# qinzheng93/GeoTransformer

Hardware: NVIDIA H100
Metric: point-cloud pairs/sec (3DMatch-shape synth) (higher is better)
Workload: dtype f32

## Files before the change

### geotransformer_b200/_lib.py

```python
import ctypes
import os
import threading

import torch

_HERE = os.path.dirname(os.path.abspath(__file__))
LIB_PATH = os.path.join(_HERE, 'libgeob200.so')
_lib = None

c_void_p, c_int64, c_int32, c_float, c_double, c_size_t, c_int = (
    ctypes.c_void_p, ctypes.c_int64, ctypes.c_int32, ctypes.c_float, ctypes.c_double, ctypes.c_size_t, ctypes.c_int)

SIGNATURES = {}


def _sig(name, restype, *argtypes):
    SIGNATURES[name] = (restype, list(argtypes))


P, I64, I32, F, D, SZ = c_void_p, c_int64, c_int32, c_float, c_double, c_size_t
_sig('geob200_last_error', ctypes.c_char_p)
_sig('geob200_launch_count', ctypes.c_uint64)
_sig('geob200_grid_subsample_workspace_bytes', SZ, I64, I64)
_sig('geob200_grid_subsample', c_int, P, I64, P, I64, F, P, P, P, SZ, P)
# ... 5 lines not shown
_sig('geob200_kpconv', c_int, P, P, P, P, I64, I64, I64, P, I64, P, P, I64, I64, F, P, P, SZ, P)
_sig('geob200_kpconv_tc_workspace_bytes', SZ, I64, I64, I64)
_sig('geob200_kpconv_tc', c_int, P, P, P, P, I64, I64, I64, P, I64, P, P, I64, I64, F, P, P, SZ, P)
_sig('geob200_set_linear_mode', None, c_int)
_sig('geob200_linear', c_int, P, I64, P, P, P, I64, I64, I64, I64, c_int, P)
_sig('geob200_split_tf32', c_int, P, I64, I64, I64, P, P)
_sig('geob200_linear_batched', c_int, P, I64, I64, P, I64, I64, P, I64, P, I64, I64, I64, I64, I64, I64, c_int, P)
_sig('geob200_group_norm_workspace_bytes', SZ, I64)
_sig('geob200_group_norm', c_int, P, I64, I64, I64, P, P, F, P, c_int, F, P, P, SZ, P)
_sig('geob200_fused_group_norm_workspace_bytes', SZ, I64, I64, I64)
_sig('geob200_linear_group_norm', c_int, P, I64, P, P, I64, I64, I64, I64, P, P, F, P, c_int, F, P, P, P, SZ, P)
_sig('geob200_kpconv_group_norm', c_int, P, P, P, P, I64, I64, I64, P, I64, P, P, I64, I64, F, I64, P, P, F, c_int, F, P, P, P, SZ,
     P, SZ, P)
_sig('geob200_group_norm_batched', c_int, P, I64, I64, I64, P, P, F, P, c_int, F, P, P, SZ, P, I64, P)
_sig('geob200_linear_group_norm_batched', c_int, P, I64, P, P, I64, I64, I64, I64, P, P, F, P, c_int, F, P, P, P, SZ, P, I64, P)
_sig('geob200_maxpool', c_int, P, P, I64, I64, I64, I64, P, P)
_sig('geob200_upsample_concat', c_int, P, P, I64, I64, P, I64, I64, I64, P, P)
_sig('geob200_kpconv_backward_workspace_bytes', SZ, I64, I64, I64, I64, I64)
_sig('geob200_kpconv_backward', c_int, P, P, P, P, I64, I64, I64, P, I64, P, I64, I64, F, P, P, P, P, P, SZ, P)
_sig('geob200_linear_backward_workspace_bytes', SZ, I64, I64, I64, c_int)
_sig('geob200_linear_backward', c_int, P, I64, P, P, I64, I64, I64, P, P, P, P, P, SZ, P)
_sig('geob200_group_norm_backward_batched_workspace_bytes', SZ, I64, I64, I64, I64)
_sig('geob200_group_norm_backward_batched', c_int, P, P, I64, I64, I64, P, F, c_int, F, P, P, P, P, P, P, SZ, P, I64, P)
_sig('geob200_maxpool_backward_batched_workspace_bytes', SZ, I64, I64, I64, I64)
_sig('geob200_maxpool_backward_batched', c_int, P, P, I64, I64, I64, I64, P, I64, P, P, P, P, SZ, P)
_sig('geob200_upsample_concat_backward_workspace_bytes', SZ, I64, I64)
_sig('geob200_upsample_concat_backward', c_int, P, I64, I64, I64, I64, I64, P, P, P, P, SZ, P)
_sig('geob200_point_to_node_partition_batched', c_int, P, P, I64, P, P, I64, P, P, P, P, P, P)
_sig('geob200_gather_rows', c_int, P, I64, I64, P, I64, P, P)
_sig('geob200_knn_partition', c_int, P, I64, P, I64, I64, P, P, P)
# ... 168 lines not shown
```

### geotransformer_b200/csrc/common.cuh

```cuda
#pragma once
#include <cuda_runtime.h>
#include <stdint.h>
#include <stdio.h>

namespace geob200 {

void set_error(const char* fmt, ...);
void count_launches(int n);
int ensure_max_smem(const void* kernel);

#define GEOB_CHECK_CUDA(expr)                                                                   \
    do {                                                                                        \
        cudaError_t _e = (expr);                                                                \
        if (_e != cudaSuccess) {                                                                \
            geob200::set_error("%s:%d CUDA error %s: %s", __FILE__, __LINE__, #expr,            \
                               cudaGetErrorString(_e));                                         \
            return -1;                                                                          \
        }                                                                                       \
    } while (0)

#define GEOB_CHECK_LAUNCH()                                                                     \
    do {                                                                                        \
        cudaError_t _e = cudaGetLastError();                                                    \
        if (_e != cudaSuccess) {                                                                \
// ... 63 lines not shown
                           int64_t n_query, int64_t n_support, int64_t n_neighbors, const float* kernel_points, int64_t n_kernel,
                           const float* weights_t, const float* bias, int64_t c_in, int64_t c_out, float sigma, int64_t groups,
                           const float* gamma, const float* beta, float eps, int leaky, float slope, float* pre_norm, float* y,
                           void* gn_workspace, size_t gn_workspace_bytes, void* workspace, size_t workspace_bytes, void* stream,
                           const GnSeg* seg, const float* w_img = nullptr);
int linear_img(const float* x, int64_t ldx, const float* weight, const float* w_img, const float* bias, float* y, int64_t ldy,
               int64_t m, int64_t n, int64_t k, int relu, void* stream);
int kpconv_tc_impl(const float* s_feats, const float* q_points, const float* s_points, const int64_t* neighbors, int64_t n_query,
                   int64_t n_support, int64_t n_neighbors, const float* kernel_points, int64_t n_kernel, const float* weights_t,
                   const float* w_img, const float* bias, int64_t c_in, int64_t c_out, float sigma, float* out, void* workspace,
                   size_t workspace_bytes, void* stream);

int maxpool_seg(const float* x, const int64_t* neighbors, int64_t n_query, int64_t n_support, int64_t n_neighbors, int64_t channels,
                float* y, const GnSeg* seg, const int* cloud_max, void* stream);

struct Segs {
    int n;
    int max;
    int start[GEOB_MAX_CLOUDS];
    int count[GEOB_MAX_CLOUDS];
};
int segs_from_counts(Segs* s, int64_t n, const int64_t* counts);
Segs segs_one(int64_t count);
Segs segs_range(const Segs& s, int first, int n);
int segs_products(Segs* s, const Segs& ref, const Segs& src);

struct Arena {
    char* base;
    size_t off;
    size_t cap;
// ... 46 lines not shown
```

### geotransformer_b200/csrc/kpconv.cu

```cuda
#include "common.cuh"
#include "geob200.h"
#include "kpconv.cuh"

namespace geob200 {

constexpr int TQ = 32;
constexpr int CC = 32;

__global__ void __launch_bounds__(256) kpconv_c1_kernel(const float* __restrict__ feats, const float* __restrict__ q_pts,
                                                        const float* __restrict__ s_pts, const long long* __restrict__ nbr,
                                                        int H, const float* __restrict__ kp, const float* __restrict__ W,
                                                        const float* __restrict__ bias, float sigma, int Ns, int M, int Cout,
                                                        float* __restrict__ out) {
    __shared__ float kp_s[KP * 3];
    __shared__ float wk_s[16][KP_PAD];
    __shared__ float np_s[16];
    if (threadIdx.x < KP * 3) kp_s[threadIdx.x] = kp[threadIdx.x];
    __syncthreads();
    const int lane = threadIdx.x & 31, warp = threadIdx.x >> 5;
    const int sub = lane >> 4, sl = lane & 15;
    const int slot = warp * 2 + sub;
    const int m = blockIdx.x * 16 + slot;
    const bool live = m < M;
    float acc[KP];
#pragma unroll
    for (int k = 0; k < KP; ++k) acc[k] = 0.f;
    int npos = 0;
    if (live) {
        const float qx = q_pts[3ll * m], qy = q_pts[3ll * m + 1], qz = q_pts[3ll * m + 2];
        for (int h = sl; h < H; h += 16) {
            const long long idx = nbr[(long long)m * H + h];
            if (idx < Ns) {
                float w[KP];
                influence15(kp_s, s_pts[3 * idx] - qx, s_pts[3 * idx + 1] - qy, s_pts[3 * idx + 2] - qz, 0.f, sigma, w);
                const float f = feats[idx];
                npos += (f > 0.f);
#pragma unroll
                for (int k = 0; k < KP; ++k) acc[k] = fmaf(w[k], f, acc[k]);
            }
        }
    }
#pragma unroll
    for (int k = 0; k < KP; ++k) {
#pragma unroll
        for (int o = 8; o > 0; o >>= 1) acc[k] += __shfl_xor_sync(0xffffffffu, acc[k], o);
    }
#pragma unroll
    for (int o = 8; o > 0; o >>= 1) npos += __shfl_xor_sync(0xffffffffu, npos, o);
    if (sl == 0) {
#pragma unroll
        for (int k = 0; k < KP; ++k) wk_s[slot][k] = acc[k];
        np_s[slot] = (float)max(npos, 1);
    }
    __syncwarp();
// ... 536 lines not shown
        sa = (red[0] + red[2]) + (red[4] + red[6]);
        sb = (red[1] + red[3]) + (red[5] + red[7]);
        const double count = (double)cpg * (double)rows;
        const double mean = sa / count;
        double var = sb / count - mean * mean;
        if (var < 0.0) var = 0.0;
        mean_rstd[((long long)p * G + g) * 2] = (float)mean;
        mean_rstd[((long long)p * G + g) * 2 + 1] = (float)(1.0 / sqrt(var + eps));
    }
}

constexpr int GN_RPB = 32;
__global__ void __launch_bounds__(256) gn_seg_apply_kernel(const float* __restrict__ x, const float* __restrict__ mean_rstd,
                                                           const float* __restrict__ gamma, const float* __restrict__ beta,
                                                           const float* __restrict__ residual, float* __restrict__ y, int n_rows,
                                                           int C, int cpg, int G, int leaky, float slope, GnSeg seg) {
    extern __shared__ float gn_tab[];
    __shared__ int starts[GEOB_MAX_CLOUDS + 1];
    for (int i = threadIdx.x; i <= seg.n_clouds; i += blockDim.x) starts[i] = seg.start[i];
    __syncthreads();
    const int r0 = blockIdx.x * GN_RPB, r1 = min(n_rows, r0 + GN_RPB);
    int c0 = 0, hi = seg.n_clouds;
    while (hi - c0 > 1) {
        const int mid = (c0 + hi) >> 1;
        if (starts[mid] <= r0) c0 = mid; else hi = mid;
    }
    for (int i = threadIdx.x; i < 2 * C; i += blockDim.x) {
        const int t = i / C, c = i % C;
        const int cl = min(c0 + t, seg.n_clouds - 1);
        const float* mr = mean_rstd + (long long)(cl % seg.n_pairs) * 2 * G + 2 * (c / cpg);
        gn_tab[(2 * t) * C + c] = mr[0];
        gn_tab[(2 * t + 1) * C + c] = mr[1];
    }
    __syncthreads();
    const int b0 = starts[c0 + 1];
    const int b1 = (c0 + 2 <= seg.n_clouds) ? starts[c0 + 2] : n_rows;
    const int C4 = C >> 2;
    const long long base4 = (long long)r0 * C4;
    const int total4 = (r1 - r0) * C4;
    for (int i = threadIdx.x; i < total4; i += blockDim.x) {
        const int row = r0 + i / C4, c = (i % C4) * 4;
        const float4 v = reinterpret_cast<const float4*>(x)[base4 + i];
        float4 rv = make_float4(0.f, 0.f, 0.f, 0.f);
        if (residual != nullptr) rv = reinterpret_cast<const float4*>(residual)[base4 + i];
        float in[4] = {v.x, v.y, v.z, v.w}, o[4];
        const float rs[4] = {rv.x, rv.y, rv.z, rv.w};
        if (row < b1) {
            const float* ta = gn_tab + (row < b0 ? 0 : 2 * C) + c;
            const float4 gm = __ldg(reinterpret_cast<const float4*>(gamma + c)), bt = __ldg(reinterpret_cast<const float4*>(beta + c));
            const float ga[4] = {gm.x, gm.y, gm.z, gm.w}, ba[4] = {bt.x, bt.y, bt.z, bt.w};
#pragma unroll
            for (int u = 0; u < 4; ++u) o[u] = (in[u] - ta[u]) * ta[C + u] * ga[u] + ba[u] + rs[u];
        } else {
            int lo = c0, hh = seg.n_clouds;
            while (hh - lo > 1) {
                const int mid = (lo + hh) >> 1;
                if (starts[mid] <= row) lo = mid; else hh = mid;
            }
            const float* mr = mean_rstd + (long long)(lo % seg.n_pairs) * 2 * G;
#pragma unroll
            for (int u = 0; u < 4; ++u) {
                const int g = (c + u) / cpg;
                o[u] = (in[u] - mr[2 * g]) * mr[2 * g + 1] * gamma[c + u] + beta[c + u] + rs[u];
            }
        }
        if (leaky) {
#pragma unroll
            for (int u = 0; u < 4; ++u) o[u] = o[u] > 0.f ? o[u] : o[u] * slope;
        }
        reinterpret_cast<float4*>(y)[base4 + i] = make_float4(o[0], o[1], o[2], o[3]);
    }
}

__global__ void __launch_bounds__(256) gn_apply_kernel(const float* __restrict__ x, const float* __restrict__ mean_rstd,
                                                       const float* __restrict__ gamma, const float* __restrict__ beta,
                                                       const float* __restrict__ residual, float* __restrict__ y,
                                                       long long total4, int C, int cpg, int leaky, float slope) {
    const long long i = (long long)blockIdx.x * blockDim.x + threadIdx.x;
    if (i >= total4) return;
    const float4 v = reinterpret_cast<const float4*>(x)[i];
    const int c = (int)((i * 4) % C);
    float in[4] = {v.x, v.y, v.z, v.w}, o[4];
    float4 rv = make_float4(0.f, 0.f, 0.f, 0.f);
    if (residual != nullptr) rv = reinterpret_cast<const float4*>(residual)[i];
    const float rs[4] = {rv.x, rv.y, rv.z, rv.w};
#pragma unroll
    for (int u = 0; u < 4; ++u) {
        const int g = (c + u) / cpg;
        float t = (in[u] - mean_rstd[2 * g]) * mean_rstd[2 * g + 1] * gamma[c + u] + beta[c + u];
        t += rs[u];
        if (leaky) t = t > 0.f ? t : t * slope;
        o[u] = t;
    }
    reinterpret_cast<float4*>(y)[i] = make_float4(o[0], o[1], o[2], o[3]);
}

__device__ __forceinline__ void maxpool_row(const float* __restrict__ x, const long long* __restrict__ nb, int W, int Ns, int C,
                                            float* __restrict__ yrow, int lane) {
    constexpr int NI = 5;
    if ((C & 3) == 0 && W <= 32 * NI) {
        int idx_l[NI];
#pragma unroll
        for (int i = 0; i < NI; ++i) idx_l[i] = (lane + 32 * i < W) ? (int)min(nb[lane + 32 * i], (long long)Ns) : Ns;
        const int C4 = C >> 2;
        for (int c0 = 0; c0 < C4; c0 += 32) {
            const int c4 = c0 + lane;
            const bool active = c4 < C4;
// ... 275 lines not shown
}

namespace geob200 {
size_t fused_group_norm_workspace_bytes_batched(int64_t n_rows, int64_t channels, int64_t groups, int64_t n_pairs) {
    return geob200_fused_group_norm_workspace_bytes(n_rows, channels, groups) + (size_t)(2 * groups * 4) * (size_t)(n_pairs > 1 ? n_pairs : 1) + 512;
}
struct GnWs { unsigned* ticket; float* mean_rstd; double* partial; };
static GnWs gn_carve(void* workspace, size_t bytes, int64_t groups, int64_t n_pairs = 1) {
    Arena ar(workspace, bytes);
    GnWs w;
    w.ticket = ar.take<unsigned>(64);
    w.mean_rstd = ar.take<float>(2 * groups * n_pairs);
    w.partial = ar.take<double>(1);
    return w;
}
static void launch_gn_seg_apply(const float* x, const GnWs& w, const float* gamma, const float* beta, const float* residual, float* y,
                                int64_t n_rows, int64_t channels, int64_t groups, float eps, int leaky, float slope, const GnSeg& seg,
                                cudaStream_t st) {
    const int cpg = (int)(channels / groups);
    const int slot_width = cpg < 32 ? cpg : 32;
    gn_seg_finalize_kernel<<<dim3((unsigned)groups, (unsigned)seg.n_pairs), 128, 0, st>>>(
        w.partial, x, (int)channels, (int)(channels / slot_width), cpg / slot_width, (int)groups, (double)eps, seg, w.mean_rstd);
    gn_seg_apply_kernel<<<(unsigned)((n_rows + GN_RPB - 1) / GN_RPB), 256, sizeof(float) * 4 * channels, st>>>(
        x, w.mean_rstd, gamma, beta, residual, y, (int)n_rows, (int)channels, cpg, (int)groups, leaky, slope, seg);
    count_launches(2);
}
static void launch_gn_tile_stats(const float* x, const GnWs& w, int64_t n_rows, int64_t channels, int64_t groups, cudaStream_t st) {
    const int cpg = (int)(channels / groups);
    const int slot_width = cpg < 32 ? cpg : 32;
    gn_tile_stats_kernel<<<(unsigned)((n_rows + 127) / 128), 256, sizeof(double) * 2 * (channels / slot_width), st>>>(
        x, (int)n_rows, (int)channels, slot_width, w.partial);
    count_launches(1);
}
static void launch_gn_apply(const float* x, const GnWs& w, const float* gamma, const float* beta, const float* residual, float* y,
                            int64_t n_rows, int64_t channels, int64_t groups, float eps, int leaky, float slope, cudaStream_t st) {
    const int cpg = (int)(channels / groups);
    const int slot_width = cpg < 32 ? cpg : 32;
    gn_finalize_kernel<<<1, 1024, 0, st>>>(w.partial, (int)((n_rows + 127) / 128), (int)(channels / slot_width), cpg / slot_width,
                                           (int)groups, (double)cpg * (double)n_rows, (double)eps, w.mean_rstd);
    const long long total4 = n_rows * channels / 4;
    gn_apply_kernel<<<(unsigned)((total4 + 255) / 256), 256, 0, st>>>(x, w.mean_rstd, gamma, beta, residual, y, total4, (int)channels,
                                                                     (int)(channels / groups), leaky, slope);
}
}

extern "C" {

int geob200_group_norm(const float* x, int64_t n_rows, int64_t channels, int64_t groups, const float* gamma,
                       const float* beta, float eps, const float* residual, int leaky, float slope, float* y,
                       void* workspace, size_t workspace_bytes, void* stream) {
    return geob200::group_norm_impl(x, n_rows, channels, groups, gamma, beta, eps, residual, leaky, slope, y, workspace, workspace_bytes,
                                    stream, nullptr);
}
}

namespace geob200 {
int group_norm_impl(const float* x, int64_t n_rows, int64_t channels, int64_t groups, const float* gamma, const float* beta, float eps,
// ... 216 lines not shown

int geob200_kpconv_group_norm_batched(const float* s_feats, const float* q_points, const float* s_points, const int64_t* neighbors,
                                      int64_t n_query, int64_t n_support, int64_t n_neighbors, const float* kernel_points, int64_t n_kernel,
                                      const float* weights_t, const float* bias, int64_t c_in, int64_t c_out, float sigma, int64_t groups,
                                      const float* gamma, const float* beta, float eps, int leaky, float slope, float* pre_norm, float* y,
                                      void* gn_workspace, size_t gn_workspace_bytes, void* workspace, size_t workspace_bytes, void* stream,
                                      int64_t n_pairs, const int64_t* cloud_rows_h) {
    geob200::GnSeg seg;
    if (geob200::make_seg(&seg, n_pairs, cloud_rows_h, n_query, "kpconv_group_norm")) return -2;
    GEOB_REQUIRE(pre_norm != nullptr && y != nullptr, "kpconv_group_norm: null output");
    return geob200::kpconv_group_norm_impl(s_feats, q_points, s_points, neighbors, n_query, n_support, n_neighbors, kernel_points, n_kernel,
                                           weights_t, bias, c_in, c_out, sigma, groups, gamma, beta, eps, leaky, slope, pre_norm, y,
                                           gn_workspace, gn_workspace_bytes, workspace, workspace_bytes, stream, &seg);
}

int geob200_maxpool_batched(const float* x, const int64_t* neighbors, int64_t n_query, int64_t n_support, int64_t n_neighbors,
                            int64_t channels, const int32_t* cloud_max, int64_t n_pairs, const int64_t* cloud_rows_h, float* y,
                            void* stream) {
    geob200::GnSeg seg;
    if (geob200::make_seg(&seg, n_pairs, cloud_rows_h, n_query, "maxpool")) return -2;
    GEOB_REQUIRE(n_query > 0 && n_support > 0 && n_neighbors > 0 && channels > 0, "maxpool: empty input");
    GEOB_REQUIRE(x != nullptr && neighbors != nullptr && cloud_max != nullptr && y != nullptr, "maxpool: null pointer");
    return geob200::maxpool_seg(x, neighbors, n_query, n_support, n_neighbors, channels, y, &seg, cloud_max, stream);
}

}
```

### geotransformer_b200/csrc/kpconv.cuh

```cuda
#pragma once
#include "common.cuh"

namespace geob200 {

constexpr int KP = 15;
constexpr int KP_PAD = 16;

__device__ __forceinline__ void influence15(const float* __restrict__ kp_s, float rx, float ry, float rz, float inv_dummy,
                                            float sigma, float* w) {
#pragma unroll
    for (int k = 0; k < KP; ++k) {
        const float dx = rx - kp_s[3 * k], dy = ry - kp_s[3 * k + 1], dz = rz - kp_s[3 * k + 2];
        const float sq = __fadd_rn(__fadd_rn(__fmul_rn(dx, dx), __fmul_rn(dy, dy)), __fmul_rn(dz, dz));
        w[k] = fmaxf(1.0f - sqrtf(sq) / sigma, 0.0f);
    }
    (void)inv_dummy;
}

__device__ __forceinline__ int cloud_of(const int* start, int n_clouds, int row) {
    int lo = 0, hi = n_clouds;
    while (hi - lo > 1) {
        const int mid = (lo + hi) >> 1;
        if (start[mid] <= row) lo = mid; else hi = mid;
    }
    return lo;
}

int make_seg(GnSeg* g, int64_t n_pairs, const int64_t* cloud_rows_h, int64_t n_rows, const char* what);

void kpconv_gather(const float* s_feats, const float* q_points, const float* s_points, const long long* neighbors, int n_neighbors,
// ... 9 lines not shown
```

### geotransformer_b200/csrc/native.cu

```cuda
#include "common.cuh"
#include "geob200.h"

namespace geob200 {

struct Ctx {
    Arena ar;
    void* gn_ws;
    size_t gn_ws_bytes;
    void* stream;
    int groups;
    Ctx(void* p, size_t n) : ar(p, n) {}
    float* fl(int64_t rows, int64_t ch) { return ar.take<float>((size_t)rows * (size_t)ch); }
};

#define TRY(expr)                  \
    do {                           \
        int _rc = (expr);          \
        if (_rc != 0) return _rc;  \
    } while (0)

static int run_kpconv(Ctx& c, const geob200_kpconv_t& k, const float* s_feats, const float* q_pts, const float* s_pts,
                      const int64_t* nbr, int64_t m, int64_t ns, int64_t h, float* out) {
    const bool tc = (k.c_in % 32 == 0) && (k.c_out % 16 == 0) && k.c_out >= 32 && (k.c_out <= 128 || k.c_out % 128 == 0) && m >= 64 &&
                    k.weights_t != nullptr;
// ... 35 lines not shown
        return 0;
    }
    TRY(run_kpconv(c, k, s_feats, q_pts, s_pts, nbr, m, ns, h, y));
    return group_norm_impl(y, m, k.c_out, c.groups, n.gamma, n.beta, 1e-5f, nullptr, 1, 0.1f, out, c.gn_ws, c.gn_ws_bytes, c.stream, seg);
}

static int run_unary(Ctx& c, const geob200_linear_t& l, const geob200_norm_t& n, const float* x, int64_t rows, const float* residual,
                     int leaky, float* out, const GnSeg* seg) {
    float* t = c.fl(rows, l.c_out);
    GEOB_REQUIRE(c.ar.ok(), "native: arena too small (unary)");
    TRY(linear_group_norm_impl(x, l.c_in, l.weight, l.bias, rows, l.c_out, l.c_in, c.groups, n.gamma, n.beta, 1e-5f, residual, leaky,
                               0.1f, t, out, c.gn_ws, c.gn_ws_bytes, c.stream, seg, l.weight_img));
    return 0;
}

static int run_resblock(Ctx& c, const geob200_resblock_t& b, const float* feats, int64_t ns, const float* q_pts, const float* s_pts,
                        const int64_t* nbr, int64_t m, int64_t h, float* out, const GnSeg* seg_s, const GnSeg* seg_q,
                        const int* cloud_max = nullptr) {
    const float* x = feats;
    if (b.has_unary1) {
        float* u = c.fl(ns, b.unary1.c_out);
        TRY(run_unary(c, b.unary1, b.norm1, feats, ns, nullptr, 1, u, seg_s));
        x = u;
    }
    float* yn = c.fl(m, b.conv.c_out);
    GEOB_REQUIRE(c.ar.ok(), "native: arena too small (resblock)");
    TRY(run_kpconv_norm(c, b.conv, b.norm_conv, x, q_pts, s_pts, nbr, m, ns, h, yn, seg_q));
    const float* sc = feats;
    if (b.strided) {
        float* mp = c.fl(m, b.c_in);
        GEOB_REQUIRE(c.ar.ok(), "native: arena too small (maxpool)");
        if (seg_q != nullptr && cloud_max != nullptr) {
            TRY(maxpool_seg(feats, nbr, m, ns, h, b.c_in, mp, seg_q, cloud_max, c.stream));
        } else {
            TRY(geob200_maxpool(feats, nbr, m, ns, h, b.c_in, mp, c.stream));
        }
        sc = mp;
    }
    if (b.has_shortcut) {
        float* s2 = c.fl(m, b.shortcut.c_out);
        TRY(run_unary(c, b.shortcut, b.norm_sc, sc, m, nullptr, 0, s2, seg_q));
        sc = s2;
    }
    return run_unary(c, b.unary2, b.norm2, yn, m, sc, 1, out, seg_q);
}

}

using namespace geob200;

extern "C" {

size_t geob200_backbone_workspace_bytes(const geob200_backbone_t* net, const int64_t* level_rows) {
    size_t total = 1 << 20;
    for (int l = 0; l < net->num_stages; ++l) {
        const size_t rows = (size_t)level_rows[l];
// ... 9 lines not shown
                                     const int64_t* const* subsampling, const int64_t* subsampling_width,
                                     const int64_t* const* upsampling, const int64_t* upsampling_width, float* const* out_feats,
                                     void* gn_workspace, size_t gn_workspace_bytes, void* workspace, size_t workspace_bytes, void* stream,
                                     int64_t n_pairs, const int64_t* const* cloud_rows_h, const int32_t* const* sub_cloud_max) {
    GEOB_REQUIRE(n_pairs == 1 || sub_cloud_max != nullptr, "backbone: batched execution needs the per-cloud subsampling widths");
    GEOB_REQUIRE(net->num_stages >= 2 && net->num_stages <= GEOB200_MAX_STAGES, "backbone: num_stages out of range");
    GEOB_REQUIRE(n_pairs >= 1 && 2 * n_pairs <= GEOB_MAX_CLOUDS, "backbone: 1 <= pairs per batch <= %d", GEOB_MAX_CLOUDS / 2);
    GEOB_REQUIRE(n_pairs == 1 || cloud_rows_h != nullptr, "backbone: batched execution needs the per-cloud row counts of every level");
    Ctx c(workspace, workspace_bytes);
    c.gn_ws = gn_workspace; c.gn_ws_bytes = gn_workspace_bytes; c.stream = stream; c.groups = net->groups;
    const int S = net->num_stages;
    GnSeg segs[GEOB200_MAX_STAGES];
    const GnSeg* sg[GEOB200_MAX_STAGES];
    for (int l = 0; l < S; ++l) {
        sg[l] = nullptr;
        if (n_pairs > 1) {
            GnSeg& g = segs[l];
            g.n_pairs = (int)n_pairs; g.n_clouds = (int)(2 * n_pairs); g.start[0] = 0;
            for (int cl = 0; cl < g.n_clouds; ++cl) g.start[cl + 1] = g.start[cl] + (int)cloud_rows_h[l][cl];
            GEOB_REQUIRE(g.start[g.n_clouds] == level_rows[l], "backbone: cloud rows of level %d do not add up", l);
            sg[l] = &g;
        }
    }
    const float* enc[GEOB200_MAX_STAGES];
    int64_t enc_ch[GEOB200_MAX_STAGES];
    {
        const int64_t n0 = level_rows[0];
        float* yn = c.fl(n0, net->conv1.c_out);
        GEOB_REQUIRE(c.ar.ok(), "native: arena too small (encoder1_1)");
        TRY(run_kpconv_norm(c, net->conv1, net->norm1, feats, points[0], points[0], neighbors[0], n0, n0, neighbor_width[0], yn, sg[0]));
        const geob200_resblock_t& b = net->blocks[0];
        float* o = c.fl(n0, b.unary2.c_out);
        TRY(run_resblock(c, b, yn, n0, points[0], points[0], neighbors[0], n0, neighbor_width[0], o, sg[0], sg[0]));
        enc[0] = o; enc_ch[0] = b.unary2.c_out;
    }
    int bi = 1;
    for (int lvl = 1; lvl < S; ++lvl) {
        const int64_t m = level_rows[lvl], ns = level_rows[lvl - 1];
        const geob200_resblock_t& b1 = net->blocks[bi++];
        float* o1 = c.fl(m, b1.unary2.c_out);
        TRY(run_resblock(c, b1, enc[lvl - 1], ns, points[lvl], points[lvl - 1], subsampling[lvl - 1], m, subsampling_width[lvl - 1], o1,
                         sg[lvl - 1], sg[lvl], sub_cloud_max != nullptr ? sub_cloud_max[lvl - 1] : nullptr));
        const geob200_resblock_t& b2 = net->blocks[bi++];
        float* o2 = c.fl(m, b2.unary2.c_out);
        TRY(run_resblock(c, b2, o1, m, points[lvl], points[lvl], neighbors[lvl], m, neighbor_width[lvl], o2, sg[lvl], sg[lvl]));
        const geob200_resblock_t& b3 = net->blocks[bi++];
        float* o3 = (lvl == S - 1) ? out_feats[0] : c.fl(m, b3.unary2.c_out);
        TRY(run_resblock(c, b3, o2, m, points[lvl], points[lvl], neighbors[lvl], m, neighbor_width[lvl], o3, sg[lvl], sg[lvl]));
        enc[lvl] = o3; enc_ch[lvl] = b3.unary2.c_out;
    }
    const float* latent = enc[S - 1];
    int64_t latent_ch = enc_ch[S - 1];
    int oi = 1;
    for (int lvl = S - 1; lvl >= net->finest_decoder; --lvl) {
        const int64_t m = level_rows[lvl - 1], ns = level_rows[lvl];
        const int64_t c2 = enc_ch[lvl - 1];
        float* cat = c.fl(m, latent_ch + c2);
        GEOB_REQUIRE(c.ar.ok(), "native: arena too small (decoder)");
        TRY(geob200_upsample_concat(latent, upsampling[lvl - 1], upsampling_width[lvl - 1], ns, enc[lvl - 1], m, latent_ch, c2, cat, stream));
        const geob200_linear_t& l = net->decoders[S - 1 - lvl];
        float* o = out_feats[oi++];
        if (lvl == net->finest_decoder) {
            TRY(linear_img(cat, l.c_in, l.weight, l.weight_img, l.bias, o, l.c_out, m, l.c_out, l.c_in, 0, stream));
// ... 113 lines not shown
```

### include/geob200.h

```cpp
#ifndef GEOB200_H
#define GEOB200_H

#include <stddef.h>
#include <stdint.h>

#ifdef __cplusplus
extern "C" {
#endif

const char* geob200_last_error(void);
uint64_t geob200_launch_count(void);


size_t geob200_grid_subsample_workspace_bytes(int64_t n_points, int64_t batch);
int geob200_grid_subsample(const float* points, int64_t n_points, const int64_t* lengths_h, int64_t batch, float voxel,
                           float* s_points, int64_t* s_lengths, void* workspace, size_t workspace_bytes, void* stream);

size_t geob200_radius_search_workspace_bytes(int64_t n_query, int64_t n_support, int64_t batch);
int geob200_radius_search(const float* q_points, int64_t n_query, const float* s_points, int64_t n_support,
                          const int64_t* q_lengths_h, const int64_t* s_lengths_h, int64_t batch, float radius,
                          int64_t width, int64_t* out, int32_t* counts, int32_t* max_count, void* workspace,
                          size_t workspace_bytes, void* stream);

int geob200_neighbor_histogram(const int64_t* neighbors, int64_t n_rows, int64_t width, int64_t n_support, int64_t hist_n,
// ... 37 lines not shown
                              void* gn_workspace, size_t gn_workspace_bytes, void* workspace, size_t workspace_bytes, void* stream);

int geob200_group_norm_batched(const float* x, int64_t n_rows, int64_t channels, int64_t groups, const float* gamma, const float* beta,
                               float eps, const float* residual, int leaky, float slope, float* y, void* workspace, size_t workspace_bytes,
                               void* stream, int64_t n_pairs, const int64_t* cloud_rows_h);
int geob200_linear_group_norm_batched(const float* x, int64_t ldx, const float* weight, const float* bias, int64_t m, int64_t n, int64_t k,
                                      int64_t groups, const float* gamma, const float* beta, float eps, const float* residual, int leaky,
                                      float slope, float* pre_norm, float* y, void* workspace, size_t workspace_bytes, void* stream,
                                      int64_t n_pairs, const int64_t* cloud_rows_h);
int geob200_kpconv_group_norm_batched(const float* s_feats, const float* q_points, const float* s_points, const int64_t* neighbors,
                                      int64_t n_query, int64_t n_support, int64_t n_neighbors, const float* kernel_points, int64_t n_kernel,
                                      const float* weights_t, const float* bias, int64_t c_in, int64_t c_out, float sigma, int64_t groups,
                                      const float* gamma, const float* beta, float eps, int leaky, float slope, float* pre_norm, float* y,
                                      void* gn_workspace, size_t gn_workspace_bytes, void* workspace, size_t workspace_bytes, void* stream,
                                      int64_t n_pairs, const int64_t* cloud_rows_h);

int geob200_maxpool(const float* x, const int64_t* neighbors, int64_t n_query, int64_t n_support, int64_t n_neighbors,
                    int64_t channels, float* y, void* stream);
int geob200_maxpool_batched(const float* x, const int64_t* neighbors, int64_t n_query, int64_t n_support, int64_t n_neighbors,
                            int64_t channels, const int32_t* cloud_max, int64_t n_pairs, const int64_t* cloud_rows_h, float* y,
                            void* stream);

int geob200_cloud_max_count(const int64_t* neighbors, int64_t n_query, int64_t n_support, int64_t n_neighbors, int64_t n_pairs,
                            const int64_t* cloud_rows_h, int32_t* cloud_max, void* stream);

int geob200_upsample_concat(const float* x, const int64_t* up_indices, int64_t up_stride, int64_t n_support,
                            const float* skip, int64_t n_query, int64_t c1, int64_t c2, float* y, void* stream);


size_t geob200_kpconv_backward_workspace_bytes(int64_t n_query, int64_t n_support, int64_t n_neighbors, int64_t c_in, int64_t c_out);
// ... 326 lines not shown
```

Measured before the change: 429.0.

## Fuse shortcut group-norm into residual apply and prefetch neighbor indices in kpconv

In each residual block the shortcut linear now computes only its output and group-norm statistics, without writing a normalized copy. Normalizing the shortcut is deferred into the unary2 group-norm apply kernel, which normalizes the residual on the fly, so one full apply pass and one intermediate buffer round-trip are dropped. The first-layer kpconv kernel also prefetches the next neighbor index, computes kernel influences inline instead of through a temporary array, and gets a minimum-blocks launch bound. The cost is extra shared memory and parameters in the apply kernel, plus possible register pressure from the launch bound.

```diff
diff --git a/geotransformer_b200/_lib.py b/geotransformer_b200/_lib.py
--- a/geotransformer_b200/_lib.py
+++ b/geotransformer_b200/_lib.py
@@ -43,6 +43,8 @@
      P, SZ, P)
 _sig('geob200_group_norm_batched', c_int, P, I64, I64, I64, P, P, F, P, c_int, F, P, P, SZ, P, I64, P)
 _sig('geob200_linear_group_norm_batched', c_int, P, I64, P, P, I64, I64, I64, I64, P, P, F, P, c_int, F, P, P, P, SZ, P, I64, P)
+_sig('geob200_linear_group_norm_stats_batched', c_int, P, I64, P, P, I64, I64, I64, I64, F, P, P, P, SZ, P, I64, P)
+_sig('geob200_group_norm_apply_batched', c_int, P, P, I64, P, P, c_int, F, P, P, I64, P, P, P, I64, I64, P, I64, P)
 _sig('geob200_maxpool', c_int, P, P, I64, I64, I64, I64, P, P)
 _sig('geob200_upsample_concat', c_int, P, P, I64, I64, P, I64, I64, I64, P, P)
 _sig('geob200_kpconv_backward_workspace_bytes', SZ, I64, I64, I64, I64, I64)
diff --git a/geotransformer_b200/csrc/common.cuh b/geotransformer_b200/csrc/common.cuh
--- a/geotransformer_b200/csrc/common.cuh
+++ b/geotransformer_b200/csrc/common.cuh
@@ -101,6 +101,35 @@
 int maxpool_seg(const float* x, const int64_t* neighbors, int64_t n_query, int64_t n_support, int64_t n_neighbors, int64_t channels,
                 float* y, const GnSeg* seg, const int* cloud_max, void* stream);
 
+__device__ __forceinline__ float gn_norm(float x, float mean, float rstd, float gamma, float beta, float residual, int leaky,
+                                         float slope) {
+    const float t = __fadd_rn(__fmaf_rn(__fmul_rn(__fsub_rn(x, mean), rstd), gamma, beta), residual);
+    return (leaky && !(t > 0.f)) ? __fmul_rn(t, slope) : t;
+}
+__device__ __forceinline__ int gn_cloud_of(const int* start, int n_clouds, int r) {
+    int lo = 0, hi = n_clouds;
+    while (hi - lo > 1) {
+        const int mid = (lo + hi) >> 1;
+        if (start[mid] <= r) lo = mid; else hi = mid;
+    }
+    return lo;
+}
+
+struct GnNorm {
+    const float* mean_rstd;
+    const float* gamma;
+    const float* beta;
+    int cpg;
+    int groups;
+    int leaky;
+    float slope;
+};
+int linear_gn_stats(const float* x, int64_t ldx, const float* weight, const float* w_img, const float* bias, int64_t m, int64_t n,
+                    int64_t k, int64_t groups, float eps, float* pre_norm, float* mean_rstd, void* workspace, size_t workspace_bytes,
+                    void* stream, const GnSeg* seg);
+int gn_apply_norm(const float* x, const GnNorm& xn, const float* residual, const GnNorm* res_norm, float* y, int64_t n_rows,
+                  int64_t channels, const GnSeg& seg, void* stream);
+
 struct Segs {
     int n;
     int max;
diff --git a/geotransformer_b200/csrc/kpconv.cu b/geotransformer_b200/csrc/kpconv.cu
--- a/geotransformer_b200/csrc/kpconv.cu
+++ b/geotransformer_b200/csrc/kpconv.cu
@@ -7,7 +7,7 @@
 constexpr int TQ = 32;
 constexpr int CC = 32;
 
-__global__ void __launch_bounds__(256) kpconv_c1_kernel(const float* __restrict__ feats, const float* __restrict__ q_pts,
+__global__ void __launch_bounds__(256, 3) kpconv_c1_kernel(const float* __restrict__ feats, const float* __restrict__ q_pts,
                                                         const float* __restrict__ s_pts, const long long* __restrict__ nbr,
                                                         int H, const float* __restrict__ kp, const float* __restrict__ W,
                                                         const float* __restrict__ bias, float sigma, int Ns, int M, int Cout,
@@ -28,16 +28,17 @@
     int npos = 0;
     if (live) {
         const float qx = q_pts[3ll * m], qy = q_pts[3ll * m + 1], qz = q_pts[3ll * m + 2];
+        long long idx = sl < H ? nbr[(long long)m * H + sl] : (long long)Ns;
         for (int h = sl; h < H; h += 16) {
-            const long long idx = nbr[(long long)m * H + h];
+            const long long next = h + 16 < H ? nbr[(long long)m * H + h + 16] : (long long)Ns;
             if (idx < Ns) {
-                float w[KP];
-                influence15(kp_s, s_pts[3 * idx] - qx, s_pts[3 * idx + 1] - qy, s_pts[3 * idx + 2] - qz, 0.f, sigma, w);
                 const float f = feats[idx];
                 npos += (f > 0.f);
-#pragma unroll
-                for (int k = 0; k < KP; ++k) acc[k] = fmaf(w[k], f, acc[k]);
-            }
+                const float rx = s_pts[3 * idx] - qx, ry = s_pts[3 * idx + 1] - qy, rz = s_pts[3 * idx + 2] - qz;
+#pragma unroll
+                for (int k = 0; k < KP; ++k) acc[k] = fmaf(influence1(kp_s, k, rx, ry, rz, sigma), f, acc[k]);
+            }
+            idx = next;
         }
     }
 #pragma unroll
@@ -604,23 +605,27 @@
 __global__ void __launch_bounds__(256) gn_seg_apply_kernel(const float* __restrict__ x, const float* __restrict__ mean_rstd,
                                                            const float* __restrict__ gamma, const float* __restrict__ beta,
                                                            const float* __restrict__ residual, float* __restrict__ y, int n_rows,
-                                                           int C, int cpg, int G, int leaky, float slope, GnSeg seg) {
+                                                           int C, int cpg, int G, int leaky, float slope, GnSeg seg,
+                                                           const float* __restrict__ r_mean_rstd, const float* __restrict__ r_gamma,
+                                                           const float* __restrict__ r_beta, int r_cpg, int r_G) {
     extern __shared__ float gn_tab[];
     __shared__ int starts[GEOB_MAX_CLOUDS + 1];
     for (int i = threadIdx.x; i <= seg.n_clouds; i += blockDim.x) starts[i] = seg.start[i];
     __syncthreads();
     const int r0 = blockIdx.x * GN_RPB, r1 = min(n_rows, r0 + GN_RPB);
-    int c0 = 0, hi = seg.n_clouds;
-    while (hi - c0 > 1) {
-        const int mid = (c0 + hi) >> 1;
-        if (starts[mid] <= r0) c0 = mid; else hi = mid;
-    }
+    const int c0 = gn_cloud_of(starts, seg.n_clouds, r0);
+    const bool rnorm = r_mean_rstd != nullptr;
     for (int i = threadIdx.x; i < 2 * C; i += blockDim.x) {
         const int t = i / C, c = i % C;
         const int cl = min(c0 + t, seg.n_clouds - 1);
         const float* mr = mean_rstd + (long long)(cl % seg.n_pairs) * 2 * G + 2 * (c / cpg);
         gn_tab[(2 * t) * C + c] = mr[0];
         gn_tab[(2 * t + 1) * C + c] = mr[1];
+        if (rnorm) {
+            const float* rr = r_mean_rstd + (long long)(cl % seg.n_pairs) * 2 * r_G + 2 * (c / r_cpg);
+            gn_tab[(4 + 2 * t) * C + c] = rr[0];
+            gn_tab[(4 + 2 * t + 1) * C + c] = rr[1];
+        }
     }
     __syncthreads();
     const int b0 = starts[c0 + 1];
@@ -634,29 +639,39 @@
         float4 rv = make_float4(0.f, 0.f, 0.f, 0.f);
         if (residual != nullptr) rv = reinterpret_cast<const float4*>(residual)[base4 + i];
         float in[4] = {v.x, v.y, v.z, v.w}, o[4];
-        const float rs[4] = {rv.x, rv.y, rv.z, rv.w};
+        float rs[4] = {rv.x, rv.y, rv.z, rv.w};
+        const float4 gm = __ldg(reinterpret_cast<const float4*>(gamma + c)), bt = __ldg(reinterpret_cast<const float4*>(beta + c));
+        const float ga[4] = {gm.x, gm.y, gm.z, gm.w}, ba[4] = {bt.x, bt.y, bt.z, bt.w};
+        float rga[4] = {0.f, 0.f, 0.f, 0.f}, rba[4] = {0.f, 0.f, 0.f, 0.f};
+        if (rnorm) {
+            const float4 rg = __ldg(reinterpret_cast<const float4*>(r_gamma + c)), rb = __ldg(reinterpret_cast<const float4*>(r_beta + c));
+            rga[0] = rg.x; rga[1] = rg.y; rga[2] = rg.z; rga[3] = rg.w;
+            rba[0] = rb.x; rba[1] = rb.y; rba[2] = rb.z; rba[3] = rb.w;
+        }
         if (row < b1) {
             const float* ta = gn_tab + (row < b0 ? 0 : 2 * C) + c;
-            const float4 gm = __ldg(reinterpret_cast<const float4*>(gamma + c)), bt = __ldg(reinterpret_cast<const float4*>(beta + c));
-            const float ga[4] = {gm.x, gm.y, gm.z, gm.w}, ba[4] = {bt.x, bt.y, bt.z, bt.w};
-#pragma unroll
-            for (int u = 0; u < 4; ++u) o[u] = (in[u] - ta[u]) * ta[C + u] * ga[u] + ba[u] + rs[u];
+            if (rnorm) {
+#pragma unroll
+                for (int u = 0; u < 4; ++u) rs[u] = gn_norm(rs[u], ta[4 * C + u], ta[5 * C + u], rga[u], rba[u], 0.f, 0, slope);
+            }
+#pragma unroll
+            for (int u = 0; u < 4; ++u) o[u] = gn_norm(in[u], ta[u], ta[C + u], ga[u], ba[u], rs[u], leaky, slope);
         } else {
-            int lo = c0, hh = seg.n_clouds;
-            while (hh - lo > 1) {
-                const int mid = (lo + hh) >> 1;
-                if (starts[mid] <= row) lo = mid; else hh = mid;
-            }
-            const float* mr = mean_rstd + (long long)(lo % seg.n_pairs) * 2 * G;
+            const int pr = gn_cloud_of(starts, seg.n_clouds, row) % seg.n_pairs;
+            const float* mr = mean_rstd + (long long)pr * 2 * G;
+            if (rnorm) {
+                const float* rr = r_mean_rstd + (long long)pr * 2 * r_G;
+#pragma unroll
+                for (int u = 0; u < 4; ++u) {
+                    const int g = (c + u) / r_cpg;
+                    rs[u] = gn_norm(rs[u], rr[2 * g], rr[2 * g + 1], rga[u], rba[u], 0.f, 0, slope);
+                }
+            }
 #pragma unroll
             for (int u = 0; u < 4; ++u) {
                 const int g = (c + u) / cpg;
-                o[u] = (in[u] - mr[2 * g]) * mr[2 * g + 1] * gamma[c + u] + beta[c + u] + rs[u];
-            }
-        }
-        if (leaky) {
-#pragma unroll
-            for (int u = 0; u < 4; ++u) o[u] = o[u] > 0.f ? o[u] : o[u] * slope;
+                o[u] = gn_norm(in[u], mr[2 * g], mr[2 * g + 1], ga[u], ba[u], rs[u], leaky, slope);
+            }
         }
         reinterpret_cast<float4*>(y)[base4 + i] = make_float4(o[0], o[1], o[2], o[3]);
     }
@@ -677,10 +692,7 @@
 #pragma unroll
     for (int u = 0; u < 4; ++u) {
         const int g = (c + u) / cpg;
-        float t = (in[u] - mean_rstd[2 * g]) * mean_rstd[2 * g + 1] * gamma[c + u] + beta[c + u];
-        t += rs[u];
-        if (leaky) t = t > 0.f ? t : t * slope;
-        o[u] = t;
+        o[u] = gn_norm(in[u], mean_rstd[2 * g], mean_rstd[2 * g + 1], gamma[c + u], beta[c + u], rs[u], leaky, slope);
     }
     reinterpret_cast<float4*>(y)[i] = make_float4(o[0], o[1], o[2], o[3]);
 }
@@ -986,16 +998,29 @@
     w.partial = ar.take<double>(1);
     return w;
 }
+static void launch_gn_seg_finalize(const float* x, const double* partial, float* mean_rstd, int64_t channels, int64_t groups, float eps,
+                                   const GnSeg& seg, cudaStream_t st) {
+    const int cpg = (int)(channels / groups);
+    const int slot_width = cpg < 32 ? cpg : 32;
+    gn_seg_finalize_kernel<<<dim3((unsigned)groups, (unsigned)seg.n_pairs), 128, 0, st>>>(
+        partial, x, (int)channels, (int)(channels / slot_width), cpg / slot_width, (int)groups, (double)eps, seg, mean_rstd);
+    count_launches(1);
+}
+static void launch_gn_seg_apply_kernel(const float* x, const GnNorm& xn, const float* residual, const GnNorm* res_norm, float* y,
+                                       int64_t n_rows, int64_t channels, const GnSeg& seg, cudaStream_t st) {
+    const size_t smem = sizeof(float) * (res_norm != nullptr ? 8 : 4) * channels;
+    gn_seg_apply_kernel<<<(unsigned)((n_rows + GN_RPB - 1) / GN_RPB), 256, smem, st>>>(
+        x, xn.mean_rstd, xn.gamma, xn.beta, residual, y, (int)n_rows, (int)channels, xn.cpg, xn.groups, xn.leaky, xn.slope, seg,
+        res_norm != nullptr ? res_norm->mean_rstd : nullptr, res_norm != nullptr ? res_norm->gamma : nullptr,
+        res_norm != nullptr ? res_norm->beta : nullptr, res_norm != nullptr ? res_norm->cpg : 1, res_norm != nullptr ? res_norm->groups : 1);
+    count_launches(1);
+}
 static void launch_gn_seg_apply(const float* x, const GnWs& w, const float* gamma, const float* beta, const float* residual, float* y,
                                 int64_t n_rows, int64_t channels, int64_t groups, float eps, int leaky, float slope, const GnSeg& seg,
                                 cudaStream_t st) {
-    const int cpg = (int)(channels / groups);
-    const int slot_width = cpg < 32 ? cpg : 32;
-    gn_seg_finalize_kernel<<<dim3((unsigned)groups, (unsigned)seg.n_pairs), 128, 0, st>>>(
-        w.partial, x, (int)channels, (int)(channels / slot_width), cpg / slot_width, (int)groups, (double)eps, seg, w.mean_rstd);
-    gn_seg_apply_kernel<<<(unsigned)((n_rows + GN_RPB - 1) / GN_RPB), 256, sizeof(float) * 4 * channels, st>>>(
-        x, w.mean_rstd, gamma, beta, residual, y, (int)n_rows, (int)channels, cpg, (int)groups, leaky, slope, seg);
-    count_launches(2);
+    launch_gn_seg_finalize(x, w.partial, w.mean_rstd, channels, groups, eps, seg, st);
+    const GnNorm xn{w.mean_rstd, gamma, beta, (int)(channels / groups), (int)groups, leaky, slope};
+    launch_gn_seg_apply_kernel(x, xn, residual, nullptr, y, n_rows, channels, seg, st);
 }
 static void launch_gn_tile_stats(const float* x, const GnWs& w, int64_t n_rows, int64_t channels, int64_t groups, cudaStream_t st) {
     const int cpg = (int)(channels / groups);
@@ -1004,15 +1029,50 @@
         x, (int)n_rows, (int)channels, slot_width, w.partial);
     count_launches(1);
 }
+static void launch_gn_finalize(const double* partial, float* mean_rstd, int64_t n_rows, int64_t channels, int64_t groups, float eps,
+                               cudaStream_t st) {
+    const int cpg = (int)(channels / groups);
+    const int slot_width = cpg < 32 ? cpg : 32;
+    gn_finalize_kernel<<<1, 1024, 0, st>>>(partial, (int)((n_rows + 127) / 128), (int)(channels / slot_width), cpg / slot_width,
+                                           (int)groups, (double)cpg * (double)n_rows, (double)eps, mean_rstd);
+}
 static void launch_gn_apply(const float* x, const GnWs& w, const float* gamma, const float* beta, const float* residual, float* y,
                             int64_t n_rows, int64_t channels, int64_t groups, float eps, int leaky, float slope, cudaStream_t st) {
-    const int cpg = (int)(channels / groups);
-    const int slot_width = cpg < 32 ? cpg : 32;
-    gn_finalize_kernel<<<1, 1024, 0, st>>>(w.partial, (int)((n_rows + 127) / 128), (int)(channels / slot_width), cpg / slot_width,
-                                           (int)groups, (double)cpg * (double)n_rows, (double)eps, w.mean_rstd);
+    launch_gn_finalize(w.partial, w.mean_rstd, n_rows, channels, groups, eps, st);
     const long long total4 = n_rows * channels / 4;
     gn_apply_kernel<<<(unsigned)((total4 + 255) / 256), 256, 0, st>>>(x, w.mean_rstd, gamma, beta, residual, y, total4, (int)channels,
                                                                      (int)(channels / groups), leaky, slope);
+}
+
+int linear_gn_stats(const float* x, int64_t ldx, const float* weight, const float* w_img, const float* bias, int64_t m, int64_t n,
+                    int64_t k, int64_t groups, float eps, float* pre_norm, float* mean_rstd, void* workspace, size_t workspace_bytes,
+                    void* stream, const GnSeg* seg) {
+    cudaStream_t st = (cudaStream_t)stream;
+    const int64_t np = (seg != nullptr && seg->n_pairs > 1) ? seg->n_pairs : 1;
+    if (g_linear_mode != 1) return 1;
+    GEOB_REQUIRE(m > 0 && n > 0 && k > 0 && groups > 0 && n % groups == 0 && n % 4 == 0, "linear_gn_stats: bad shape");
+    GEOB_REQUIRE(workspace_bytes >= (np > 1 ? fused_group_norm_workspace_bytes_batched(m, n, groups, np)
+                                            : geob200_fused_group_norm_workspace_bytes(m, n, groups)), "linear_gn_stats: workspace too small");
+    const GnWs w = gn_carve(workspace, workspace_bytes, groups, np);
+    GnFuse gn{(int)groups, 0, w.partial};
+    const int rc = linear_tc(x, ldx, weight, k, w_img, bias, nullptr, pre_norm, n, m, n, k, 0, st, &gn);
+    if (rc != 0) return rc;
+    if (np > 1) launch_gn_seg_finalize(pre_norm, w.partial, mean_rstd, n, groups, eps, *seg, st);
+    else {
+        launch_gn_finalize(w.partial, mean_rstd, m, n, groups, eps, st);
+        count_launches(1);
+    }
+    GEOB_CHECK_LAUNCH();
+    return 0;
+}
+
+int gn_apply_norm(const float* x, const GnNorm& xn, const float* residual, const GnNorm* res_norm, float* y, int64_t n_rows,
+                  int64_t channels, const GnSeg& seg, void* stream) {
+    GEOB_REQUIRE(n_rows > 0 && channels % 4 == 0 && seg.start[seg.n_clouds] == n_rows, "gn_apply_norm: bad shape");
+    if (res_norm != nullptr && sizeof(float) * 8 * channels > 48 * 1024 && ensure_max_smem((const void*)gn_seg_apply_kernel)) return -1;
+    launch_gn_seg_apply_kernel(x, xn, residual, res_norm, y, n_rows, channels, seg, (cudaStream_t)stream);
+    GEOB_CHECK_LAUNCH();
+    return 0;
 }
 }
 
@@ -1259,6 +1319,32 @@
                                            gn_workspace, gn_workspace_bytes, workspace, workspace_bytes, stream, &seg);
 }
 
+
+int geob200_linear_group_norm_stats_batched(const float* x, int64_t ldx, const float* weight, const float* bias, int64_t m, int64_t n,
+                                            int64_t k, int64_t groups, float eps, float* pre_norm, float* mean_rstd, void* workspace,
+                                            size_t workspace_bytes, void* stream, int64_t n_pairs, const int64_t* cloud_rows_h) {
+    geob200::GnSeg seg;
+    if (geob200::make_seg(&seg, n_pairs, cloud_rows_h, m, "linear_group_norm_stats")) return -2;
+    const int rc = geob200::linear_gn_stats(x, ldx, weight, nullptr, bias, m, n, k, groups, eps, pre_norm, mean_rstd, workspace,
+                                            workspace_bytes, stream, &seg);
+    GEOB_REQUIRE(rc <= 0, "linear_group_norm_stats: the statistics of this shape do not come from the tensor-core GEMM epilogue");
+    return rc;
+}
+
+int geob200_group_norm_apply_batched(const float* x, const float* mean_rstd, int64_t groups, const float* gamma, const float* beta,
+                                     int leaky, float slope, const float* residual, const float* res_mean_rstd, int64_t res_groups,
+                                     const float* res_gamma, const float* res_beta, float* y, int64_t n_rows, int64_t channels,
+                                     void* stream, int64_t n_pairs, const int64_t* cloud_rows_h) {
+    geob200::GnSeg seg;
+    if (geob200::make_seg(&seg, n_pairs, cloud_rows_h, n_rows, "group_norm_apply")) return -2;
+    GEOB_REQUIRE(groups > 0 && channels % groups == 0 && (res_mean_rstd == nullptr || (res_groups > 0 && channels % res_groups == 0)),
+                 "group_norm_apply: bad group count");
+    const geob200::GnNorm xn{mean_rstd, gamma, beta, (int)(channels / groups), (int)groups, leaky, slope};
+    const geob200::GnNorm rn{res_mean_rstd, res_gamma, res_beta, res_mean_rstd != nullptr ? (int)(channels / res_groups) : 1,
+                             (int)res_groups, 0, slope};
+    return geob200::gn_apply_norm(x, xn, residual, res_mean_rstd != nullptr ? &rn : nullptr, y, n_rows, channels, seg, stream);
+}
+
 int geob200_maxpool_batched(const float* x, const int64_t* neighbors, int64_t n_query, int64_t n_support, int64_t n_neighbors,
                             int64_t channels, const int32_t* cloud_max, int64_t n_pairs, const int64_t* cloud_rows_h, float* y,
                             void* stream) {
diff --git a/geotransformer_b200/csrc/kpconv.cuh b/geotransformer_b200/csrc/kpconv.cuh
--- a/geotransformer_b200/csrc/kpconv.cuh
+++ b/geotransformer_b200/csrc/kpconv.cuh
@@ -6,14 +6,15 @@
 constexpr int KP = 15;
 constexpr int KP_PAD = 16;
 
+__device__ __forceinline__ float influence1(const float* __restrict__ kp_s, int k, float rx, float ry, float rz, float sigma) {
+    const float dx = rx - kp_s[3 * k], dy = ry - kp_s[3 * k + 1], dz = rz - kp_s[3 * k + 2];
+    const float sq = __fadd_rn(__fadd_rn(__fmul_rn(dx, dx), __fmul_rn(dy, dy)), __fmul_rn(dz, dz));
+    return fmaxf(1.0f - sqrtf(sq) / sigma, 0.0f);
+}
 __device__ __forceinline__ void influence15(const float* __restrict__ kp_s, float rx, float ry, float rz, float inv_dummy,
                                             float sigma, float* w) {
 #pragma unroll
-    for (int k = 0; k < KP; ++k) {
-        const float dx = rx - kp_s[3 * k], dy = ry - kp_s[3 * k + 1], dz = rz - kp_s[3 * k + 2];
-        const float sq = __fadd_rn(__fadd_rn(__fmul_rn(dx, dx), __fmul_rn(dy, dy)), __fmul_rn(dz, dz));
-        w[k] = fmaxf(1.0f - sqrtf(sq) / sigma, 0.0f);
-    }
+    for (int k = 0; k < KP; ++k) w[k] = influence1(kp_s, k, rx, ry, rz, sigma);
     (void)inv_dummy;
 }
 
diff --git a/geotransformer_b200/csrc/native.cu b/geotransformer_b200/csrc/native.cu
--- a/geotransformer_b200/csrc/native.cu
+++ b/geotransformer_b200/csrc/native.cu
@@ -73,8 +73,25 @@
     return 0;
 }
 
+static int run_unary_stats(Ctx& c, const geob200_linear_t& l, const geob200_norm_t& n, const float* x, int64_t rows, int leaky,
+                           const GnSeg* seg, const GnSeg& lk, const float** t, GnNorm* pn) {
+    const size_t mark = c.ar.off;
+    float* pre = c.fl(rows, l.c_out);
+    float* mr = c.fl(2 * (int64_t)c.groups * lk.n_pairs, 1);
+    GEOB_REQUIRE(c.ar.ok(), "native: arena too small (unary)");
+    const int rc = linear_gn_stats(x, l.c_in, l.weight, l.weight_img, l.bias, rows, l.c_out, l.c_in, c.groups, 1e-5f, pre, mr, c.gn_ws,
+                                   c.gn_ws_bytes, c.stream, seg);
+    if (rc != 0) {
+        c.ar.off = mark;
+        return rc;
+    }
+    *t = pre;
+    *pn = GnNorm{mr, n.gamma, n.beta, (int)(l.c_out / c.groups), c.groups, leaky, 0.1f};
+    return 0;
+}
+
 static int run_resblock(Ctx& c, const geob200_resblock_t& b, const float* feats, int64_t ns, const float* q_pts, const float* s_pts,
-                        const int64_t* nbr, int64_t m, int64_t h, float* out, const GnSeg* seg_s, const GnSeg* seg_q,
+                        const int64_t* nbr, int64_t m, int64_t h, float* out, const GnSeg* seg_s, const GnSeg* seg_q, const GnSeg& lk,
                         const int* cloud_max = nullptr) {
     const float* x = feats;
     if (b.has_unary1) {
@@ -96,9 +113,27 @@
         }
         sc = mp;
     }
+    GnNorm scn{};
+    bool sc_pending = false;
     if (b.has_shortcut) {
+        const int rc = run_unary_stats(c, b.shortcut, b.norm_sc, sc, m, 0, seg_q, lk, &sc, &scn);
+        if (rc < 0) return rc;
+        sc_pending = rc == 0;
+        if (!sc_pending) {
+            float* s2 = c.fl(m, b.shortcut.c_out);
+            TRY(run_unary(c, b.shortcut, b.norm_sc, sc, m, nullptr, 0, s2, seg_q));
+            sc = s2;
+        }
+    }
+    const float* t2 = nullptr;
+    GnNorm n2{};
+    const int rc = run_unary_stats(c, b.unary2, b.norm2, yn, m, 1, seg_q, lk, &t2, &n2);
+    if (rc < 0) return rc;
+    if (rc == 0) return gn_apply_norm(t2, n2, sc, sc_pending ? &scn : nullptr, out, m, b.unary2.c_out, lk, c.stream);
+    if (sc_pending) {
         float* s2 = c.fl(m, b.shortcut.c_out);
-        TRY(run_unary(c, b.shortcut, b.norm_sc, sc, m, nullptr, 0, s2, seg_q));
+        GEOB_REQUIRE(c.ar.ok(), "native: arena too small (shortcut)");
+        TRY(gn_apply_norm(sc, scn, nullptr, nullptr, s2, m, b.shortcut.c_out, lk, c.stream));
         sc = s2;
     }
     return run_unary(c, b.unary2, b.norm2, yn, m, sc, 1, out, seg_q);
@@ -138,6 +173,7 @@
     const GnSeg* sg[GEOB200_MAX_STAGES];
     for (int l = 0; l < S; ++l) {
         sg[l] = nullptr;
+        segs[l].n_pairs = 1; segs[l].n_clouds = 1; segs[l].start[0] = 0; segs[l].start[1] = (int)level_rows[l];
         if (n_pairs > 1) {
             GnSeg& g = segs[l];
             g.n_pairs = (int)n_pairs; g.n_clouds = (int)(2 * n_pairs); g.start[0] = 0;
@@ -155,7 +191,7 @@
         TRY(run_kpconv_norm(c, net->conv1, net->norm1, feats, points[0], points[0], neighbors[0], n0, n0, neighbor_width[0], yn, sg[0]));
         const geob200_resblock_t& b = net->blocks[0];
         float* o = c.fl(n0, b.unary2.c_out);
-        TRY(run_resblock(c, b, yn, n0, points[0], points[0], neighbors[0], n0, neighbor_width[0], o, sg[0], sg[0]));
+        TRY(run_resblock(c, b, yn, n0, points[0], points[0], neighbors[0], n0, neighbor_width[0], o, sg[0], sg[0], segs[0]));
         enc[0] = o; enc_ch[0] = b.unary2.c_out;
     }
     int bi = 1;
@@ -164,13 +200,13 @@
         const geob200_resblock_t& b1 = net->blocks[bi++];
         float* o1 = c.fl(m, b1.unary2.c_out);
         TRY(run_resblock(c, b1, enc[lvl - 1], ns, points[lvl], points[lvl - 1], subsampling[lvl - 1], m, subsampling_width[lvl - 1], o1,
-                         sg[lvl - 1], sg[lvl], sub_cloud_max != nullptr ? sub_cloud_max[lvl - 1] : nullptr));
+                         sg[lvl - 1], sg[lvl], segs[lvl], sub_cloud_max != nullptr ? sub_cloud_max[lvl - 1] : nullptr));
         const geob200_resblock_t& b2 = net->blocks[bi++];
         float* o2 = c.fl(m, b2.unary2.c_out);
-        TRY(run_resblock(c, b2, o1, m, points[lvl], points[lvl], neighbors[lvl], m, neighbor_width[lvl], o2, sg[lvl], sg[lvl]));
+        TRY(run_resblock(c, b2, o1, m, points[lvl], points[lvl], neighbors[lvl], m, neighbor_width[lvl], o2, sg[lvl], sg[lvl], segs[lvl]));
         const geob200_resblock_t& b3 = net->blocks[bi++];
         float* o3 = (lvl == S - 1) ? out_feats[0] : c.fl(m, b3.unary2.c_out);
-        TRY(run_resblock(c, b3, o2, m, points[lvl], points[lvl], neighbors[lvl], m, neighbor_width[lvl], o3, sg[lvl], sg[lvl]));
+        TRY(run_resblock(c, b3, o2, m, points[lvl], points[lvl], neighbors[lvl], m, neighbor_width[lvl], o3, sg[lvl], sg[lvl], segs[lvl]));
         enc[lvl] = o3; enc_ch[lvl] = b3.unary2.c_out;
     }
     const float* latent = enc[S - 1];
diff --git a/include/geob200.h b/include/geob200.h
--- a/include/geob200.h
+++ b/include/geob200.h
@@ -75,6 +75,14 @@
                                       const float* gamma, const float* beta, float eps, int leaky, float slope, float* pre_norm, float* y,
                                       void* gn_workspace, size_t gn_workspace_bytes, void* workspace, size_t workspace_bytes, void* stream,
                                       int64_t n_pairs, const int64_t* cloud_rows_h);
+
+int geob200_linear_group_norm_stats_batched(const float* x, int64_t ldx, const float* weight, const float* bias, int64_t m, int64_t n,
+                                            int64_t k, int64_t groups, float eps, float* pre_norm, float* mean_rstd, void* workspace,
+                                            size_t workspace_bytes, void* stream, int64_t n_pairs, const int64_t* cloud_rows_h);
+int geob200_group_norm_apply_batched(const float* x, const float* mean_rstd, int64_t groups, const float* gamma, const float* beta,
+                                     int leaky, float slope, const float* residual, const float* res_mean_rstd, int64_t res_groups,
+                                     const float* res_gamma, const float* res_beta, float* y, int64_t n_rows, int64_t channels,
+                                     void* stream, int64_t n_pairs, const int64_t* cloud_rows_h);
 
 int geob200_maxpool(const float* x, const int64_t* neighbors, int64_t n_query, int64_t n_support, int64_t n_neighbors,
                     int64_t channels, float* y, void* stream);
```

After: 442.0 (median of 6 runs). +3.0%, better.
